# saandeepa93/distributed_compute_pytorch

Measured on AMD Instinct MI355X. Metric: samples/sec (whole node) ResNet-50 DDP at 1/2/4/8 MI355X; scaling efficiency, higher is better.
Workload: dtype bf16; 1 GPU; model=resnet50, global_batch=1024, per_gpu_batch=1024, grad_accum=1, parallelism=dp1, impl=ours, fused_kernels=True, optimizer=SGD, comm_dtype=fp32, hip_graph=False, grad_to_none=True, backend=rccl, mfma_1x1_gemm=True, image_size=224, channels_last=True, res_prologue=False

## Files before the change

### csrc/fused.cpp

```cpp
#include "fused.h"

#include <cstring>

#include <c10/hip/HIPGuard.h>
#include <c10/hip/HIPStream.h>

#include <map>
#include <tuple>
#include <mutex>

#include "common.h"
#include "kernels/bn_kernels.h"
#include "kernels/gemm_kernels.h"
#include "kernels/attn_kernels.h"
#include "kernels/kernels.h"
#include "kernels/ln_kernels.h"
#include "kernels/dropout_kernels.h"
#include "kernels/pool_kernels.h"
#include "kernels/metrics_kernels.h"
#include "kernels/gelu_kernels.h"

namespace dcp {
namespace fused {

// ... 25 lines not shown

struct ZeroArena {
  at::Tensor buf;
  int64_t used = 0;
};
std::mutex g_arena_mu;
std::map<std::pair<int, hipStream_t>, ZeroArena> g_arenas;
constexpr int64_t kArenaFloats = int64_t(4) << 20;

at::Tensor zeroed_floats(int64_t n, const at::Tensor& like, hipStream_t st) {
  hipStreamCaptureStatus cap = hipStreamCaptureStatusNone;
  (void)hipStreamIsCapturing(st, &cap);
  const int64_t need = (n + 63) / 64 * 64;
  if (cap != hipStreamCaptureStatusNone || need > kArenaFloats / 4) {
    return at::zeros({need}, like.options().dtype(at::kFloat)).narrow(0, 0, n);
  }
  std::lock_guard<std::mutex> g(g_arena_mu);
  ZeroArena& a = g_arenas[{static_cast<int>(like.get_device()), st}];
  if (!a.buf.defined()) {
    a.buf = at::empty({kArenaFloats}, like.options().dtype(at::kFloat));
    DK_CHECK(hipMemsetAsync(a.buf.data_ptr(), 0, sizeof(float) * kArenaFloats, st) == hipSuccess, "memset failed");
  }
  if (a.used + need > kArenaFloats) {
    DK_CHECK(hipMemsetAsync(a.buf.data_ptr(), 0, sizeof(float) * kArenaFloats, st) == hipSuccess, "memset failed");
    a.used = 0;
  }
  at::Tensor t = a.buf.narrow(0, a.used, n);
  a.used += need;
  return t;
}

at::Tensor zeroed_vec(int64_t n, const at::Tensor& like, hipStream_t st) {
  constexpr int64_t kSlab = int64_t(1) << 18;
  hipStreamCaptureStatus cap = hipStreamCaptureStatusNone;
  (void)hipStreamIsCapturing(st, &cap);
  const int64_t need = (n + 63) / 64 * 64;
  static const bool off = std::getenv("DCP_NO_GRAD_SLAB") != nullptr;
  if (off || need > kSlab / 4) return at::zeros({n}, like.options().dtype(at::kFloat));
  static std::mutex mu;
  if (cap != hipStreamCaptureStatusNone) {
    unsigned long long id = 0;
    (void)hipStreamGetCaptureInfo(st, &cap, &id);
    static std::map<std::pair<int, hipStream_t>, std::tuple<at::Tensor, int64_t, unsigned long long>> cslabs;
    std::lock_guard<std::mutex> g(mu);
    auto& e = cslabs[{static_cast<int>(like.get_device()), st}];
    if (!std::get<0>(e).defined() || std::get<2>(e) != id || std::get<1>(e) + need > kSlab) {
// ... 643 lines not shown
            "conv1x1_dgrad_resred: mean must be fp32 [N]");
  DK_CHECK(bits.scalar_type() == at::kByte && bits.numel() == M * N / 8 && bits.is_contiguous(),
            "conv1x1_dgrad_resred: relu bits mismatch");
  at::Tensor g2;
  if (gy2.has_value() && gy2->defined()) {
    g2 = gy2->to(at::kBFloat16).contiguous(x.dim() == 4 ? at::MemoryFormat::ChannelsLast : at::MemoryFormat::Contiguous);
    DK_CHECK(g2.sizes() == x.sizes(), "conv1x1_dgrad_resred: gy2 shape");
  }
  const bool has_x2 = x2.has_value() && x2->defined();
  if (has_x2) {
    check_gemm_act(*x2, "conv1x1_dgrad_resred(x2)");
    DK_CHECK(x2->sizes() == x.sizes(), "conv1x1_dgrad_resred: x2 shape");
    DK_CHECK(mean2.has_value() && mean2->defined() && mean2->scalar_type() == at::kFloat && mean2->numel() == N,
              "conv1x1_dgrad_resred: mean2 must be fp32 [N]");
  }
  at::Tensor g = at::empty_like(x, x.dim() == 4 ? at::MemoryFormat::ChannelsLast : at::MemoryFormat::Contiguous);
  auto s = stream_of(gy);
  at::Tensor acc = zeroed_floats(2 * N, gy, s);
  at::Tensor acc2 = has_x2 ? zeroed_floats(2 * N, gy, s) : at::empty({0}, gy.options().dtype(at::kFloat));
  kern::gemm_nt_resred_bf16(gy.data_ptr(), wt.data_ptr(), g.data_ptr(), M, static_cast<int>(N), static_cast<int>(K),
                            x.data_ptr(), mean.data_ptr<float>(), g2.defined() ? g2.data_ptr() : nullptr,
                            bits.data_ptr<uint8_t>(), acc.data_ptr<float>(), has_x2 ? x2->data_ptr() : nullptr,
                            has_x2 ? mean2->data_ptr<float>() : nullptr, has_x2 ? acc2.data_ptr<float>() : nullptr, s);
  return {g, acc, acc2};
}

std::vector<at::Tensor> conv3_bwd_fused(const at::Tensor& g, const at::Tensor& z3, const at::Tensor& gamma3,
                                        const at::Tensor& mean3, const at::Tensor& invstd3, const at::Tensor& acc3,
                                        const at::Tensor& wt, const at::Tensor& x2,
                                        const c10::optional<at::Tensor>& gamma2,
                                        const c10::optional<at::Tensor>& beta2, const at::Tensor& mean2,
                                        const at::Tensor& invstd2) {
  check_gemm_act(g, "conv3_bwd_fused");
  check_gemm_act(z3, "conv3_bwd_fused");
  c10::hip::HIPGuard guard(g.device().index());
  DK_CHECK(g.dim() == 4 && g.sizes() == z3.sizes(), "conv3_bwd_fused: g must match z3");
  const int64_t C = g.size(1);
  const int64_t M = g.numel() / C;
  const int64_t w = C / 4;
  DK_CHECK(C % 4 == 0 && kern::conv3_bwd_mode(M, static_cast<int>(w)) > 0, "conv3_bwd_fused: unsupported shape");
  DK_CHECK(wt.scalar_type() == at::kBFloat16 && wt.is_contiguous() && wt.numel() == w * C,
            "conv3_bwd_fused: weight must be contiguous bf16 [w][4w]");
  auto f32c = [&](const at::Tensor& t, int64_t n) {
    return t.scalar_type() == at::kFloat && t.numel() == n && t.is_contiguous() && t.device() == g.device();
  };
  DK_CHECK(f32c(gamma3, C) && f32c(mean3, C) && f32c(invstd3, C) && f32c(acc3, 2 * C),
// ... 1077 lines not shown
        pybind11::arg("accumulate_into") = pybind11::none());
  m.def("flash_attn_fwd", &flash_attn_fwd, "MFMA flash attention forward (head dim 64)", pybind11::arg("q"),
        pybind11::arg("k"), pybind11::arg("v"), pybind11::arg("heads"), pybind11::arg("causal"),
        pybind11::arg("p_drop"), pybind11::arg("seed"), pybind11::arg("keep_bits") = true,
        pybind11::arg("key_mask") = pybind11::none(), pybind11::kw_only(),
        pybind11::arg("seed_offset") = pybind11::none());
  m.def("flash_attn_bwd", &flash_attn_bwd, "MFMA flash attention backward into dq/dk/dv", pybind11::arg("dout"),
        pybind11::arg("q"), pybind11::arg("k"), pybind11::arg("v"), pybind11::arg("o"), pybind11::arg("lse"),
        pybind11::arg("keep"), pybind11::arg("heads"), pybind11::arg("causal"), pybind11::arg("p_drop"),
        pybind11::arg("seed"), pybind11::arg("dq"), pybind11::arg("dk"), pybind11::arg("dv"),
        pybind11::arg("key_mask") = pybind11::none());
  m.def("attn_pack_key_mask", &attn_pack_key_mask,
        "bool [B, T] key-padding mask -> packed int64 [B, 1 + T/64] for flash_attn_fwd / flash_attn_bwd",
        pybind11::arg("mask"));
  m.def("conv_fwd", &conv_fwd, "kxk NHWC conv forward (implicit-GEMM MFMA) [+ output BN sums]", pybind11::arg("x"),
        pybind11::arg("wt"), pybind11::arg("kh"), pybind11::arg("kw"), pybind11::arg("stride"), pybind11::arg("pad"),
        pybind11::arg("stats") = false);
  m.def("conv1x1_dgrad_bnred", &conv1x1_dgrad_bnred, "1x1 data gradient + BN/ReLU backward reduction epilogue");
  m.def("conv_dgrad_bnred", &conv_dgrad_bnred, "stride-1 kxk data gradient + BN/ReLU backward reduction epilogue");
  m.def("conv1x1_dgrad_resred", &conv1x1_dgrad_resred,
        "1x1 data gradient + residual BN(+RBN)/ReLU backward reduction epilogue -> (g, acc, acc2)",
        pybind11::arg("gy"), pybind11::arg("wt"), pybind11::arg("x"), pybind11::arg("gy2"), pybind11::arg("mean"),
        pybind11::arg("bits"), pybind11::arg("x2") = pybind11::none(), pybind11::arg("mean2") = pybind11::none());
  m.def("bn_bwd_apply_g", &bn_bwd_apply_g, "BN training backward apply from a masked gradient + its reduction");
  m.def("conv3_bwd_fused", &conv3_bwd_fused,
        "bottleneck conv3 backward with BN3's backward apply as its prologue -> (dy2, acc2, dz3)");
  m.def("conv3_bwd_mode", [](int64_t M, int64_t w) { return kern::conv3_bwd_mode(M, static_cast<int>(w)); },
        "0: conv3's backward of this shape stays unfused; 1: conv3_bwd_fused");
  m.def("conv3_bwd_ds_fused", &conv3_bwd_ds_fused,
        "conv3_bwd_fused at a downsample block: both BNs' backward applies as the prologue -> "
        "(dy2, acc2, dz3, dzd[, dxd])");
  m.def("conv3_bwd_ds_mode", [](int64_t M, int64_t w) { return kern::conv3_bwd_ds_mode(M, static_cast<int>(w)); },
        "0: a downsample block of this shape stays on bn_bwd_apply2_g; 1: conv3_bwd_ds_fused without dxd; 2: with");
  m.def("bn_dparams", &bn_dparams, "(dweight, dbias) of a training BN from its backward reduction");
  m.def("conv1_fwd_fused", &conv1_fwd_fused,
        "block boundary relu(bn3(z3) + residual-or-bn_d(x2)) with the next conv1 fed from the same tile -> "
        "(y, bits, z1, sums1, mean, invstd[, mean2, invstd2])",
        pybind11::arg("z3"), pybind11::arg("w"), pybind11::arg("weight"), pybind11::arg("bias"),
        pybind11::arg("running_mean"), pybind11::arg("running_var"), pybind11::arg("num_batches_tracked"),
        pybind11::arg("stats"), pybind11::arg("momentum"), pybind11::arg("eps"),
        pybind11::arg("residual") = pybind11::none(), pybind11::arg("x2") = pybind11::none(),
        pybind11::arg("weight2") = pybind11::none(), pybind11::arg("bias2") = pybind11::none(),
        pybind11::arg("running_mean2") = pybind11::none(), pybind11::arg("running_var2") = pybind11::none(),
        pybind11::arg("num_batches_tracked2") = pybind11::none(), pybind11::arg("stats2") = pybind11::none(),
        pybind11::arg("momentum2") = 0.0, pybind11::arg("eps2") = 0.0);
  m.def("conv1_fwd_mode",
// ... 38 lines not shown
```

### csrc/kernels/gemm.hip

```cpp
#include <hip/hip_runtime.h>

#include <cstdlib>
#include <string>

#include "bf16_vec.h"
#include "gelu_math.h"
#include "gemm_kernels.h"
#include "kernels.h"
#include "stem_kernels.h"

namespace dcp {
namespace kern {
namespace {

typedef short s16x4 __attribute__((ext_vector_type(4)));
typedef short s16x8 __attribute__((ext_vector_type(8)));
typedef __attribute__((address_space(3))) s16x4 lds_s16x4;

constexpr int kT = 256;
int g_wg_slots = 512;
int g_wg_cap = 0;
constexpr int kBK = 32;
constexpr int kNS = 4;

// ... 1568 lines not shown
  const char* v = getenv("DCP_RESERVE_CUS");
  const int r = v ? atoi(v) : 0;
  return r < 0 ? 0 : (r > 192 ? 192 : r);
}();
inline int grid_cus() { return 256 - g_reserve_cus; }
}
void gemm_tune(const char* key, int value) {
  const std::string k(key);
  if (k == "nt_big") g_nt_big = value;
  if (k == "lin_big") g_lin_big = value;
  if (k == "big_pipe") g_big_pipe = value;
  if (k == "nt_a") g_nt_a = value < 0 ? 0 : (value > 3 ? 3 : value);
  if (k == "stem_wide") g_stem_wide = value;
  if (k == "slab32") g_slab32 = value;
  if (k == "nt_deep") g_nt_deep = value;
  if (k == "pro_pipe") g_pro_pipe = value;
  if (k == "wg_slots") g_wg_slots = value < 64 ? 64 : value;
  if (k == "wg_cap") g_wg_cap = value < 0 ? 0 : value;
  if (k == "reserve_cus") g_reserve_cus = value < 0 ? 0 : (value > 192 ? 192 : value);
  if (k.rfind("pp_", 0) == 0) gemm_pp_tune(key, value);
  if (k.rfind("bn_", 0) == 0) bn_tune(key, value);
  if (k.rfind("c3bwd", 0) == 0) conv3_bwd_tune(key, value);
  if (k.rfind("c1fwd", 0) == 0) conv1_fwd_tune(key, value);
  wgrad_pp_tune(key, value);
}
int gemm_tune_get(const char* key) {
  const std::string k(key);
  if (k == "nt_big") return g_nt_big;
  if (k == "lin_big") return g_lin_big;
  if (k == "big_pipe") return g_big_pipe;
  if (k == "nt_a") return g_nt_a;
  if (k == "stem_wide") return g_stem_wide;
  if (k == "slab32") return g_slab32;
  if (k == "nt_deep") return g_nt_deep;
  if (k == "pro_pipe") return g_pro_pipe;
  if (k == "wg_slots") return g_wg_slots;
  if (k == "wg_cap") return g_wg_cap;
  if (k == "reserve_cus") return g_reserve_cus;
  if (k.rfind("pp_", 0) == 0) return gemm_pp_tune_get(key);
  if (k.rfind("bn_", 0) == 0) return bn_tune_get(key);
  if (k.rfind("c3bwd", 0) == 0) return conv3_bwd_tune_get(key);
  if (k.rfind("c1fwd", 0) == 0) return conv1_fwd_tune_get(key);
  return wgrad_pp_tune_get(key);
}

namespace {
template <bool GATHER, int BK, int BM>
void gemm_nt_launch_bm(const void* A, const void* B, void* C, int64_t M, int N, int K, const float* scale,
                       const float* shift, bool relu, float* stats, const ConvGeo& geo, const BnRedArgs* red,
                       hipStream_t s, bool scatter2, bool parity) {
  const int BN = N % 128 == 0 ? 128 : 64;
  const int tiles_m = static_cast<int>((M + BM - 1) / BM);
  const int tn = N / BN;
  const int kRes = (BM == 128 ? 2 : 1) * grid_cus();
  const int64_t tiles = static_cast<int64_t>(tiles_m) * tn;
  int P = tiles <= kRes ? static_cast<int>(tiles) : (kRes / tn) * tn;
  if (P < tn) P = tn;
  const dim3 grid(P);
  const bool pro = scale != nullptr;
  const bool st = stats != nullptr;
  const int nw = (BM / 64) * (BN == 64 && BM == 256 ? 1 : 2);
  const size_t lds = static_cast<size_t>(nt_stages<BK>()) * (BM + BN) * BK * 2 +
                     static_cast<size_t>(nw) * 32 * (BN * 2 / (BM == 256 && BN == 64 ? 1 : 2)) +
                     (pro ? 8 * static_cast<size_t>(K) : 0);
  const int NT = 64 * nw;
// ... 831 lines not shown
```

### csrc/kernels/kernels.h

```cpp
#pragma once

#include <hip/hip_runtime.h>

#include <cstdint>

namespace dcp {
namespace kern {

enum DType : int { F32 = 0, BF16 = 1, F16 = 2 };

constexpr int64_t kChunk = 8192;

struct TableView {
  const int64_t* base;
  int n;
};

void mt_copy(TableView t, int64_t nchunks, DType src, DType dst, float scale, hipStream_t s);

void mt_sgd(TableView t, int64_t nchunks, DType p, float lr, float momentum, float dampening, float wd,
            bool nesterov, bool maximize, bool first_step, bool has_buf, float grad_scale, hipStream_t s);

void mt_adam(TableView t, int64_t nchunks, DType p, float lr, float beta1, float beta2, float eps, float wd,
             float bias_c1, float bias_c2_sqrt, bool amsgrad, bool decoupled_wd, bool maximize, float grad_scale,
// ... 15 lines not shown

void conv3_bwd_bf16(const void* g, const void* z3, const void* wt, const void* x2, void* dz3, void* dy2, int64_t M,
                    int w, const float* gamma3, const float* mean3, const float* invstd3, const float* acc3,
                    const float* gamma2, const float* beta2, const float* mean2, const float* invstd2, float* stats,
                    hipStream_t s);
int conv3_bwd_mode(int64_t M, int w);
void conv3_bwd_ds_bf16(const void* g, const void* z3, const void* zd, const void* wt, const void* wdt, const void* x2,
                       void* dz3, void* dzd, void* dy2, void* dxd, int64_t M, int w, const float* gamma3,
                       const float* mean3, const float* invstd3, const float* acc3, const float* gammad,
                       const float* meand, const float* invstdd, const float* accd, const float* gamma2,
                       const float* beta2, const float* mean2, const float* invstd2, float* stats, hipStream_t s);
int conv3_bwd_ds_mode(int64_t M, int w);
bool conv3_bwd_tune(const char* key, int value);
int conv3_bwd_tune_get(const char* key);
void bn_dparams(const float* acc, const float* invstd, float* dgamma, float* dbeta, int C, hipStream_t s);

void conv1_fwd_bf16(const void* z3, const void* res, const void* w, void* y, uint8_t* bits, void* z1, int64_t M, int K,
                    int N, const float* scale, const float* shift, const float* rscale, const float* rshift,
                    float* stats, hipStream_t s);
int conv1_fwd_mode(int64_t M, int K, int N);
bool conv1_fwd_tune(const char* key, int value);
int conv1_fwd_tune_get(const char* key);

}
}
```

### csrc/selftest/kern_stubs.cpp

```cpp
#include <cstdio>
#include <cstdlib>

#include "kernels/kernels.h"

namespace dcp {
namespace kern {
namespace {
[[noreturn]] void gpu_only(const char* f) {
  std::fprintf(stderr, "%s: GPU launcher reached from a CPU self-test\n", f);
  std::abort();
}
}

void mt_copy(TableView, int64_t, DType, DType, float, hipStream_t) { gpu_only("mt_copy"); }
void mt_sgd(TableView, int64_t, DType, float, float, float, float, bool, bool, bool, bool, float, hipStream_t) {
  gpu_only("mt_sgd");
}
void mt_adam(TableView, int64_t, DType, float, float, float, float, float, float, float, bool, bool, bool, float, bool,
             int, hipStream_t) {
  gpu_only("mt_adam");
}
void mt_adadelta(TableView, int64_t, DType, float, float, float, float, bool, float, hipStream_t) {
  gpu_only("mt_adadelta");
}
// ... 3 lines not shown
void conv3_bwd_bf16(const void*, const void*, const void*, const void*, void*, void*, int64_t, int, const float*,
                    const float*, const float*, const float*, const float*, const float*, const float*, const float*,
                    float*, hipStream_t) {
  gpu_only("conv3_bwd_bf16");
}
int conv3_bwd_mode(int64_t, int) { return 0; }
void conv3_bwd_ds_bf16(const void*, const void*, const void*, const void*, const void*, const void*, void*, void*,
                       void*, void*, int64_t, int, const float*, const float*, const float*, const float*,
                       const float*, const float*, const float*, const float*, const float*, const float*,
                       const float*, const float*, float*, hipStream_t) {
  gpu_only("conv3_bwd_ds_bf16");
}
int conv3_bwd_ds_mode(int64_t, int) { return 0; }
bool conv3_bwd_tune(const char*, int) { return false; }
int conv3_bwd_tune_get(const char*) { return -1; }
void bn_dparams(const float*, const float*, float*, float*, int, hipStream_t) { gpu_only("bn_dparams"); }
void conv1_fwd_bf16(const void*, const void*, const void*, void*, uint8_t*, void*, int64_t, int, int, const float*,
                    const float*, const float*, const float*, float*, hipStream_t) {
  gpu_only("conv1_fwd_bf16");
}
int conv1_fwd_mode(int64_t, int, int) { return 0; }
bool conv1_fwd_tune(const char*, int) { return false; }
int conv1_fwd_tune_get(const char*) { return -1; }

}
}
```

### distributed_compute_pytorch_amd/ops/conv.py

```python
from __future__ import annotations

from typing import Optional, Tuple

import torch
import torch.nn.functional as F

from .._ext import C as _C


def _cl(t: torch.Tensor) -> torch.Tensor:
    if t.dtype != torch.bfloat16:
        t = t.to(torch.bfloat16)
    return t.contiguous(memory_format=torch.channels_last) if t.dim() == 4 else t.contiguous()


_PREPPED = {}


class ConvWeightPrep:

    def __init__(self, weights):
        self.weights = list(weights)
        self._key = None

# ... 175 lines not shown
def _c3_defer_ok(z3: torch.Tensor) -> bool:
    fn = _c3_node(z3)
    c = z3.shape[1]
    if fn is None or _C.conv3_bwd_mode(z3.numel() // c, c // 4) <= 0:
        return False
    fn._c3_defer = True
    return True


def _c3ds_defer_ok(z3: torch.Tensor, zd: torch.Tensor):
    fn, fd = _c3_node(z3), zd.grad_fn
    if (fn is None or fd is None or fd is fn or not _APPLY2 or zd.shape != z3.shape or zd.dtype != z3.dtype
            or not zd.is_contiguous(memory_format=torch.channels_last)):
        return None
    c = z3.shape[1]
    mode = _C.conv3_bwd_ds_mode(z3.numel() // c, c // 4)
    if mode == 2:
        if not isinstance(fd, _Conv1x1Fn._backward_cls) or tuple(fd.wshape) != (c, c // 4, 1, 1):
            return None
    elif mode != 1 or not isinstance(fd, (_Conv1x1Fn._backward_cls, _ConvKxKGemmFn._backward_cls)):
        return None
    fn._c3ds = fd._c3ds = True
    return fn, fd, mode == 2


_PRO_RED = True


class _BNReluConv1x1Fn(torch.autograd.Function):
    @staticmethod
    def forward(ctx, x, gamma, beta, weight, running_mean, running_var, nbt, momentum, eps, stats, sums):
        mean, invstd, scale, shift = _C.bn_stats_coef(x, gamma, beta, running_mean, running_var, float(momentum),
                                                      float(eps), nbt, sums)
        w, wt = _w2d(weight)
        z, st = _C.conv1x1_fwd(x, w, scale, shift, True, bool(stats))
        ctx.save_for_backward(x, gamma, beta, wt, mean, invstd, scale, shift)
        ctx.wshape, ctx.wdtype = weight.shape, weight.dtype
        ctx.mark_non_differentiable(st)
        ctx.set_materialize_grads(False)
        return z, st

    @staticmethod
    def backward(ctx, gz, _gst):
        x, gamma, beta, wt, mean, invstd, scale, shift = ctx.saved_tensors
        if gz is None:
            return (None,) * 11
# ... 84 lines not shown
            w, wt = _w2d(w_next)
            z1, s1 = _C.conv1x1_fwd(y, w, None, None, False, True)
        elif RES_PROLOGUE:
            mean, invstd, scale, shift = _C.bn_stats_coef(z3, gamma, beta, rm, rv, float(momentum), float(eps), nbt,
                                                          stats)
            w, wt = _w2d(w_next)
            z1, s1, y, bits = _C.conv1x1_fwd_res(z3, w, scale, shift, _cl(residual), True)
            mean2 = invstd2 = None
        else:
            y, mean, invstd, bits = _C.bn_act_fwd(z3, gamma, beta, rm, rv, residual, True, float(momentum),
                                                  float(eps), True, nbt, stats)
            mean2 = invstd2 = None
            w, wt = _w2d(w_next)
            z1, s1 = _C.conv1x1_fwd(y, w, None, None, False, True)
        ctx.save_for_backward(z3, gamma, mean, invstd, bits, y, wt, x2, gamma2, mean2, invstd2)
        ctx.wshape, ctx.wdtype = w_next.shape, w_next.dtype
        ctx.mark_non_differentiable(s1)
        return y, z1, s1

    @staticmethod
    def backward(ctx, gy, gz, _gs):
        z3, gamma, mean, invstd, bits, y, wt, x2, gamma2, mean2, invstd2 = ctx.saved_tensors
        if gz is None:
            gz = torch.zeros((y.shape[0], ctx.wshape[0]) + tuple(y.shape[2:]), device=y.device, dtype=y.dtype)
        gz = _cl(gz)
        dw = _C.conv1x1_wgrad(gz, y)
        g, acc, acc2 = _C.conv1x1_dgrad_resred(gz, wt, z3, None if gy is None else _cl(gy), mean, bits, x2, mean2)
        dres = dx2 = dgamma2 = dbeta2 = None
        if x2 is not None and _APPLY2 and ctx.defer_ds:
            _c3ds_put(g, (z3, gamma, mean, invstd, acc, x2, gamma2, mean2, invstd2, acc2), ctx.defer_ds)
            dz3 = dx2 = g
            dgamma, dbeta = _C.bn_dparams(acc, invstd)
            dgamma2, dbeta2 = _C.bn_dparams(acc2, invstd2)
        elif x2 is not None and _APPLY2:
            dz3, dgamma, dbeta, dx2, dgamma2, dbeta2 = _C.bn_bwd_apply2_g(g, z3, gamma, mean, invstd, acc, x2, gamma2,
                                                                          mean2, invstd2, acc2)
        elif ctx.defer:
            _c3_put(g, z3, gamma, mean, invstd, acc)
            dz3 = dres = g
            dgamma, dbeta = _C.bn_dparams(acc, invstd)
        else:
            dz3, dgamma, dbeta = _C.bn_bwd_apply_g(g, z3, gamma, mean, invstd, acc)
            if x2 is not None:
                dx2, dgamma2, dbeta2 = _C.bn_bwd_apply_g(g, x2, gamma2, mean2, invstd2, acc2)
            else:
                dres = g
        dw = dw.view(ctx.wshape)
        if dw.dtype != ctx.wdtype:
            dw = dw.to(ctx.wdtype)
        return (dz3, dgamma, dbeta, dres, dx2, dgamma2, dbeta2, dw) + (None,) * 13
# ... 64 lines not shown
        d3 = _c3_take(ctx, gz)
        ds = _c3ds_take(ctx, gz, 0)
        if d3 is not None or ds is not None:
            dy, acc, gz = (_C.conv3_bwd_fused(gz, *d3, wt, x, gamma, beta, mean, invstd) if d3 is not None
                           else ds[:3])
            dw = _C.conv1x1_wgrad(gz, y).view(wshape)
        elif k == 1 and stride == 1:
            dw = _C.conv1x1_wgrad(gz, y).view(wshape)
            dy, acc = _C.conv1x1_dgrad_bnred(gz, wt, x, gamma, beta, mean, invstd)
        else:
            dw = _C.conv_wgrad(gz, y, k, k, stride, pad)
            if stride == 1:
                wd = wt if wt is not None else w.flip(2, 3).permute(1, 2, 3, 0).contiguous()
                dy, acc = _C.conv_dgrad_bnred(gz, wd, k, k, k - 1 - pad, x, gamma, beta, mean, invstd)
            else:
                dy = torch.ops.aten.convolution_backward(gz, y, w, None, [stride, stride], [pad, pad], [1, 1],
                                                         False, [0, 0], 1, [True, False, False])[0]
                dy = _cl(dy)
                acc = None
        if dw.dtype != wdtype:
            dw = dw.to(wdtype)
        if acc is None:
            dx, dgamma, dbeta, _ = _C.bn_act_bwd(dy, None, x, gamma, beta, mean, invstd, y, True, False, True, None)
        else:
            dx, dgamma, dbeta = _C.bn_act_bwd_apply(dy, x, gamma, beta, mean, invstd, acc)
        return dx, dgamma, dbeta, dw, None, None, None, None, None, None, None, None, None, None


def bn_relu_conv(x: torch.Tensor, bn, weight: torch.Tensor, k: int, stride: int, pad: int,
                 sums: Optional[torch.Tensor] = None, stats: bool = False):
    nbt = bn.num_batches_tracked
    if nbt is not None and (nbt.device != x.device or nbt.dtype != torch.int64):
        nbt.add_(1)
        nbt = None
    return _BNReluConvFn.apply(x, bn.weight, bn.bias, weight, bn.running_mean, bn.running_var, nbt, bn.momentum,
                               bn.eps, sums, k, stride, pad, stats)


class _ConvKxKFn(torch.autograd.Function):

    @staticmethod
    def forward(ctx, x, weight, stride, padding):
        w = weight.detach().to(torch.bfloat16)
        y = F.conv2d(x, w, None, stride, padding)
        ctx.save_for_backward(x, w)
        ctx.stride, ctx.padding, ctx.wdtype = stride, padding, weight.dtype
        return y

    @staticmethod
    def backward(ctx, gy):
        x, w = ctx.saved_tensors
        gy = _cl(gy)
        s, p = ctx.stride, ctx.padding
        dx = None
        if ctx.needs_input_grad[0]:
            dx = torch.ops.aten.convolution_backward(gy, x, w, None, [s, s], [p, p], [1, 1], False, [0, 0], 1,
                                                     [True, False, False])[0]
        dw = None
        if ctx.needs_input_grad[1]:
# ... 92 lines not shown
```

Baseline: 15650 samples/s.

## Add streaming conv1 backward kernel with optional deferred BN1 apply prologue

Adds a new row-tile streaming MFMA kernel for the 1x1 conv1 data gradient at bottleneck boundaries. It fuses the residual BN/ReLU reduction epilogue and can take BN1's backward apply as a prologue, deferring that apply from the bn_relu_conv node through a Python-side handoff. The aim is fewer kernel launches and fewer activation round-trips through HBM in the backward pass. BN1 fusion is off by default (g_bn1=0), so only the streaming dgrad kernel runs for the 64x256 and 128x512 shapes. The arena reset now reallocates its buffer instead of re-zeroing in place, which avoids overwriting slices still in use at the cost of an extra allocation.

```diff
diff --git a/csrc/fused.cpp b/csrc/fused.cpp
--- a/csrc/fused.cpp
+++ b/csrc/fused.cpp
@@ -71,6 +71,7 @@
     DK_CHECK(hipMemsetAsync(a.buf.data_ptr(), 0, sizeof(float) * kArenaFloats, st) == hipSuccess, "memset failed");
   }
   if (a.used + need > kArenaFloats) {
+    a.buf = at::empty({kArenaFloats}, like.options().dtype(at::kFloat));
     DK_CHECK(hipMemsetAsync(a.buf.data_ptr(), 0, sizeof(float) * kArenaFloats, st) == hipSuccess, "memset failed");
     a.used = 0;
   }
@@ -760,6 +761,75 @@
                             x.data_ptr(), mean.data_ptr<float>(), g2.defined() ? g2.data_ptr() : nullptr,
                             bits.data_ptr<uint8_t>(), acc.data_ptr<float>(), has_x2 ? x2->data_ptr() : nullptr,
                             has_x2 ? mean2->data_ptr<float>() : nullptr, has_x2 ? acc2.data_ptr<float>() : nullptr, s);
+  return {g, acc, acc2};
+}
+
+std::vector<at::Tensor> conv1_bwd_fused(const at::Tensor& gy, const at::Tensor& wt, const at::Tensor& x,
+                                        const c10::optional<at::Tensor>& gy2, const at::Tensor& mean,
+                                        const at::Tensor& bits, const c10::optional<at::Tensor>& x2,
+                                        const c10::optional<at::Tensor>& mean2, const c10::optional<at::Tensor>& z1,
+                                        const c10::optional<at::Tensor>& gamma1,
+                                        const c10::optional<at::Tensor>& beta1,
+                                        const c10::optional<at::Tensor>& mean1,
+                                        const c10::optional<at::Tensor>& invstd1,
+                                        const c10::optional<at::Tensor>& acc1) {
+  check_gemm_act(gy, "conv1_bwd_fused");
+  check_gemm_act(x, "conv1_bwd_fused");
+  c10::hip::HIPGuard guard(gy.device().index());
+  DK_CHECK(gy.dim() == 4 && x.dim() == 4, "conv1_bwd_fused: gy and x must be channels_last 4-D tensors");
+  const int64_t K = gy.size(1), N = x.size(1);
+  const int64_t M = gy.numel() / K;
+  const int mode = kern::conv1_bwd_mode(M, static_cast<int>(K), static_cast<int>(N));
+  DK_CHECK(mode > 0, "conv1_bwd_fused: unsupported shape");
+  DK_CHECK(wt.scalar_type() == at::kBFloat16 && wt.is_contiguous() && wt.numel() == N * K &&
+                wt.device() == gy.device(),
+            "conv1_bwd_fused: weight must be contiguous bf16 [N][K]");
+  DK_CHECK(x.numel() == M * N && x.size(0) == gy.size(0) && x.device() == gy.device(), "conv1_bwd_fused: x shape");
+  auto f32c = [&](const at::Tensor& t, int64_t n) {
+    return t.scalar_type() == at::kFloat && t.numel() == n && t.is_contiguous() && t.device() == gy.device();
+  };
+  DK_CHECK(f32c(mean, N), "conv1_bwd_fused: mean must be fp32 [N]");
+  DK_CHECK(bits.scalar_type() == at::kByte && bits.numel() == M * N / 8 && bits.is_contiguous() &&
+                bits.device() == gy.device(),
+            "conv1_bwd_fused: relu bits mismatch");
+  at::Tensor g2;
+  if (gy2.has_value() && gy2->defined()) {
+    g2 = gy2->to(at::kBFloat16).contiguous(at::MemoryFormat::ChannelsLast);
+    DK_CHECK(g2.sizes() == x.sizes() && g2.device() == gy.device(), "conv1_bwd_fused: gy2 shape");
+  }
+  const bool has_x2 = x2.has_value() && x2->defined();
+  if (has_x2) {
+    check_gemm_act(*x2, "conv1_bwd_fused(x2)");
+    DK_CHECK(x2->sizes() == x.sizes() && x2->device() == gy.device(), "conv1_bwd_fused: x2 shape");
+    DK_CHECK(mean2.has_value() && mean2->defined() && f32c(*mean2, N), "conv1_bwd_fused: mean2 must be fp32 [N]");
+  }
+  const bool bn1 = z1.has_value() && z1->defined();
+  BnRedIn r1;
+  if (bn1) {
+    DK_CHECK(mode == 2, "conv1_bwd_fused: BN1 fusion is switched off (gemm_tune c1bwd_bn1)");
+    DK_CHECK(mean1.has_value() && mean1->defined() && invstd1.has_value() && invstd1->defined() &&
+                  acc1.has_value() && acc1->defined() && f32c(*mean1, K) && f32c(*invstd1, K) && f32c(*acc1, 2 * K),
+              "conv1_bwd_fused: BN1 mean / invstd fp32 [K], acc fp32 [2*K]");
+    r1 = bnred_in(*z1, gamma1, beta1, *mean1, *invstd1, K, "conv1_bwd_fused(z1)");
+    DK_CHECK(z1->sizes() == gy.sizes() && z1->device() == gy.device(), "conv1_bwd_fused: z1 must match gy");
+    DK_CHECK((!r1.w.defined() || f32c(r1.w, K)) && (!r1.b.defined() || f32c(r1.b, K)),
+              "conv1_bwd_fused: BN1 gamma / beta [K]");
+  }
+  at::Tensor g = at::empty_like(x, at::MemoryFormat::ChannelsLast);
+  at::Tensor dz1;
+  if (bn1) dz1 = at::empty_like(gy, at::MemoryFormat::ChannelsLast);
+  auto s = stream_of(gy);
+  at::Tensor acc = zeroed_floats(2 * N, gy, s);
+  at::Tensor acc2 = has_x2 ? zeroed_floats(2 * N, gy, s) : at::empty({0}, gy.options().dtype(at::kFloat));
+  kern::conv1_bwd_bf16(gy.data_ptr(), wt.data_ptr(), g.data_ptr(), M, static_cast<int>(N), static_cast<int>(K),
+                       x.data_ptr(), mean.data_ptr<float>(), g2.defined() ? g2.data_ptr() : nullptr,
+                       bits.data_ptr<uint8_t>(), acc.data_ptr<float>(), has_x2 ? x2->data_ptr() : nullptr,
+                       has_x2 ? mean2->data_ptr<float>() : nullptr, has_x2 ? acc2.data_ptr<float>() : nullptr,
+                       bn1 ? z1->data_ptr() : nullptr, bn1 && r1.w.defined() ? r1.w.data_ptr<float>() : nullptr,
+                       bn1 && r1.b.defined() ? r1.b.data_ptr<float>() : nullptr, bn1 ? r1.mean : nullptr,
+                       bn1 ? r1.invstd : nullptr, bn1 ? acc1->data_ptr<float>() : nullptr,
+                       bn1 ? dz1.data_ptr() : nullptr, s);
+  if (bn1) return {g, acc, acc2, dz1};
   return {g, acc, acc2};
 }
 
@@ -1883,6 +1953,18 @@
         "1x1 data gradient + residual BN(+RBN)/ReLU backward reduction epilogue -> (g, acc, acc2)",
         pybind11::arg("gy"), pybind11::arg("wt"), pybind11::arg("x"), pybind11::arg("gy2"), pybind11::arg("mean"),
         pybind11::arg("bits"), pybind11::arg("x2") = pybind11::none(), pybind11::arg("mean2") = pybind11::none());
+  m.def("conv1_bwd_fused", &conv1_bwd_fused,
+        "conv1x1_dgrad_resred on the streaming row-tile kernel -> (g, acc, acc2); with z1 … acc1 BN1's backward "
+        "apply is its prologue (gy = dy1) -> (g, acc, acc2, dz1)",
+        pybind11::arg("gy"), pybind11::arg("wt"), pybind11::arg("x"), pybind11::arg("gy2"), pybind11::arg("mean"),
+        pybind11::arg("bits"), pybind11::arg("x2") = pybind11::none(), pybind11::arg("mean2") = pybind11::none(),
+        pybind11::arg("z1") = pybind11::none(), pybind11::arg("gamma1") = pybind11::none(),
+        pybind11::arg("beta1") = pybind11::none(), pybind11::arg("mean1") = pybind11::none(),
+        pybind11::arg("invstd1") = pybind11::none(), pybind11::arg("acc1") = pybind11::none());
+  m.def("conv1_bwd_mode",
+        [](int64_t M, int64_t K, int64_t N) { return kern::conv1_bwd_mode(M, static_cast<int>(K), static_cast<int>(N)); },
+        "0: conv1's boundary data gradient of this shape stays on conv1x1_dgrad_resred; 1: conv1_bwd_fused; "
+        "2: and BN1's backward apply may be deferred into it");
   m.def("bn_bwd_apply_g", &bn_bwd_apply_g, "BN training backward apply from a masked gradient + its reduction");
   m.def("conv3_bwd_fused", &conv3_bwd_fused,
         "bottleneck conv3 backward with BN3's backward apply as its prologue -> (dy2, acc2, dz3)");
diff --git a/csrc/kernels/conv1_bwd.hip b/csrc/kernels/conv1_bwd.hip
--- /dev/null
+++ b/csrc/kernels/conv1_bwd.hip
@@ -0,0 +1,346 @@
+#include <hip/hip_runtime.h>
+
+#include <cstring>
+
+#include "bf16_vec.h"
+#include "kernels.h"
+
+namespace dcp {
+namespace kern {
+namespace {
+
+constexpr int kBM = 32;
+
+int g_mode64 = 1;
+int g_mode128 = 1;
+int g_mode128x256 = 0;
+int g_bn1 = 0;
+int g_grid = 0;
+
+struct C1BArgs {
+  const uint16_t* a;
+  const uint16_t* z1;
+  uint16_t* dz1;
+  const uint16_t* wt;
+  const uint16_t* z3;
+  const uint16_t* gy2;
+  const uint8_t* bits;
+  const uint16_t* x2;
+  uint16_t* g;
+  const float* mean3;
+  const float* meand;
+  float* acc;
+  float* acc2;
+  const float* gamma1;
+  const float* beta1;
+  const float* mean1;
+  const float* invstd1;
+  const float* acc1;
+  int64_t M;
+  int tiles;
+};
+
+template <int K, int N, bool X2, bool BN1>
+__global__ void __launch_bounds__(4 * K, 2) conv1_bwd_kernel(const C1BArgs a) {
+  constexpr int T = 4 * K;
+  constexpr int NW = T / 64;
+  constexpr int WN = N / NW;
+  constexpr int FN = WN / 16;
+  constexpr int FM = kBM / 16;
+  constexpr int KS = K / 32;
+  constexpr int ACH = K / 8;
+  constexpr int CPR = N / 8;
+  constexpr int RPP = T / CPR;
+  constexpr int NP = kBM / RPP;
+  static_assert(T == kBM * ACH && RPP * NP == kBM && FN * 16 * NW == N && CPR >= 16, "tile shape");
+  __shared__ __attribute__((aligned(16))) char sA[kBM * K * 2];
+  __shared__ __attribute__((aligned(16))) char sC[kBM * N * 2];
+  static_assert(RPP * N * 4 <= kBM * N * 2, "sums fit the staging image");
+  __shared__ __attribute__((aligned(16))) float sK[BN1 ? 6 * K : 4];
+
+  const int t = threadIdx.x, lane = t & 63, wv = t >> 6;
+  const int cc = t % CPR, r0 = t / CPR;
+  const int ach = t % ACH, arow = t / ACH;
+  const int64_t M = a.M;
+  const bool has2 = a.gy2 != nullptr;
+
+  const int P = gridDim.x, wg = xcd_remap(blockIdx.x, P);
+
+  if constexpr (BN1) {
+    for (int c = t; c < K; c += T) {
+      const float inv = a.invstd1[c];
+      const float sb = a.acc1[c], sg = a.acc1[K + c];
+      const float m = a.mean1[c];
+      const float sc = (a.gamma1 ? a.gamma1[c] : 1.f) * inv;
+      sK[c] = sc;
+      sK[K + c] = sb / static_cast<float>(M);
+      sK[2 * K + c] = sg / static_cast<float>(M) * inv * inv;
+      sK[3 * K + c] = m;
+      sK[4 * K + c] = sc;
+      sK[5 * K + c] = (a.beta1 ? a.beta1[c] : 0.f) - m * sc;
+    }
+    __syncthreads();
+  }
+  bf16x8 wf[FN][KS];
+#pragma unroll
+  for (int i = 0; i < FN; ++i) {
+    const uint16_t* wp = a.wt + static_cast<int64_t>(WN * wv + 16 * i + (lane & 15)) * K + 8 * (lane >> 4);
+#pragma unroll
+    for (int ks = 0; ks < KS; ++ks) wf[i][ks] = *reinterpret_cast<const bf16x8*>(wp + 32 * ks);
+  }
+  float rmu[8], rmu2[X2 ? 8 : 1], ssum[8], ssq[8], ss2[X2 ? 8 : 1];
+#pragma unroll
+  for (int k = 0; k < 8; ++k) {
+    rmu[k] = a.mean3[cc * 8 + k];
+    if constexpr (X2) {
+      rmu2[k] = a.meand[cc * 8 + k];
+      ss2[k] = 0.f;
+    }
+    ssum[k] = ssq[k] = 0.f;
+  }
+
+  uint4 aq, zq1;
+  auto load_a = [&](int tl) {
+    const int64_t m0 = static_cast<int64_t>(tl) * kBM;
+    const int rem = static_cast<int>(M - m0 < kBM ? M - m0 : kBM);
+    const uint32_t lo = (arow < rem ? arow : 0) * K + ach * 8;
+    aq = ld16_nt(a.a + m0 * K + lo);
+    if constexpr (BN1) zq1 = ld16_nt(a.z1 + m0 * K + lo);
+  };
+  uint4 zq[NP], gq[NP], xq[X2 ? NP : 1];
+  uint32_t bq[NP];
+  auto load_e = [&](int tl, int i) {
+    const int64_t m0 = static_cast<int64_t>(tl) * kBM;
+    const int rem = static_cast<int>(M - m0 < kBM ? M - m0 : kBM);
+    const int row = r0 + RPP * i;
+    const uint32_t lo = (row < rem ? row : 0) * N + cc * 8;
+    zq[i] = ld16_nt(a.z3 + m0 * N + lo);
+    if (has2) gq[i] = ld16_nt(a.gy2 + m0 * N + lo);
+    bq[i] = __builtin_nontemporal_load(a.bits + (m0 * N >> 3) + (lo >> 3));
+    if constexpr (X2) xq[i] = ld16_nt(a.x2 + m0 * N + lo);
+  };
+#pragma unroll
+  for (int i = 0; i < NP; ++i) gq[i] = make_uint4(0, 0, 0, 0);
+
+  int tl = wg;
+  if (tl < a.tiles) {
+    load_a(tl);
+#pragma unroll
+    for (int i = 0; i < NP; ++i) load_e(tl, i);
+  }
+  for (; tl < a.tiles; tl += P) {
+    const int64_t m0 = static_cast<int64_t>(tl) * kBM;
+    const bool more = tl + P < a.tiles;
+    {
+      uint4 v = aq;
+      if constexpr (BN1) {
+        const uint32_t g4[4] = {aq.x, aq.y, aq.z, aq.w};
+        const uint32_t z4[4] = {zq1.x, zq1.y, zq1.z, zq1.w};
+        float k1[8], k2[8], k3[8], mu[8], sc[8], sf[8], d[8];
+#pragma unroll
+        for (int h = 0; h < 2; ++h) {
+          const float* kp = sK + ach * 8 + 4 * h;
+          *reinterpret_cast<float4*>(k1 + 4 * h) = *reinterpret_cast<const float4*>(kp);
+          *reinterpret_cast<float4*>(k2 + 4 * h) = *reinterpret_cast<const float4*>(kp + K);
+          *reinterpret_cast<float4*>(k3 + 4 * h) = *reinterpret_cast<const float4*>(kp + 2 * K);
+          *reinterpret_cast<float4*>(mu + 4 * h) = *reinterpret_cast<const float4*>(kp + 3 * K);
+          *reinterpret_cast<float4*>(sc + 4 * h) = *reinterpret_cast<const float4*>(kp + 4 * K);
+          *reinterpret_cast<float4*>(sf + 4 * h) = *reinterpret_cast<const float4*>(kp + 5 * K);
+        }
+#pragma unroll
+        for (int k = 0; k < 8; ++k) {
+          float gk = (k & 1) ? bf_hi(g4[k >> 1]) : bf_lo(g4[k >> 1]);
+          const float xk = (k & 1) ? bf_hi(z4[k >> 1]) : bf_lo(z4[k >> 1]);
+          gk = fmaf(xk, sc[k], sf[k]) > 0.f ? gk : 0.f;
+          d[k] = k1[k] * (gk - k2[k] - (xk - mu[k]) * k3[k]);
+        }
+        v = make_uint4(pack2(d[0], d[1]), pack2(d[2], d[3]), pack2(d[4], d[5]), pack2(d[6], d[7]));
+        if (m0 + arow < M) st16_nt(a.dz1 + (m0 + arow) * K + ach * 8, v);
+      }
+      if (m0 + arow >= M) v = make_uint4(0, 0, 0, 0);
+      const int sw = ACH >= 16 ? (arow & 15) : ((arow >> 1) & 7);
+      *reinterpret_cast<uint4*>(sA + arow * (K * 2) + 16 * (ach ^ sw)) = v;
+    }
+    __syncthreads();
+    if (more) load_a(tl + P);
+
+    f32x4 acc[FN][FM];
+#pragma unroll
+    for (int i = 0; i < FN; ++i)
+#pragma unroll
+      for (int j = 0; j < FM; ++j) acc[i][j] = f32x4{0.f, 0.f, 0.f, 0.f};
+#pragma unroll
+    for (int ks = 0; ks < KS; ++ks) {
+      bf16x8 xf[FM];
+#pragma unroll
+      for (int j = 0; j < FM; ++j) {
+        const int row = 16 * j + (lane & 15);
+        const int sw = ACH >= 16 ? (row & 15) : ((row >> 1) & 7);
+        xf[j] = *reinterpret_cast<const bf16x8*>(sA + row * (K * 2) + 16 * ((4 * ks + (lane >> 4)) ^ sw));
+      }
+#pragma unroll
+      for (int i = 0; i < FN; ++i)
+#pragma unroll
+        for (int j = 0; j < FM; ++j)
+          acc[i][j] = __builtin_amdgcn_mfma_f32_16x16x32_bf16(wf[i][ks], xf[j], acc[i][j], 0, 0, 0);
+    }
+#pragma unroll
+    for (int j = 0; j < FM; ++j) {
+      const int row = 16 * j + (lane & 15);
+#pragma unroll
+      for (int i = 0; i < FN; ++i) {
+        const int col = WN * wv + 16 * i + 4 * (lane >> 4);
+        *reinterpret_cast<uint2*>(sC + row * (N * 2) + 16 * ((col >> 3) ^ (row & 15)) + (col & 7) * 2) =
+            make_uint2(pack2(acc[i][j][0], acc[i][j][1]), pack2(acc[i][j][2], acc[i][j][3]));
+      }
+    }
+    __syncthreads();
+
+#pragma unroll
+    for (int i = 0; i < NP; ++i) {
+      const int row = r0 + RPP * i;
+      const int64_t m = m0 + row;
+      const uint4 v = *reinterpret_cast<const uint4*>(sC + row * (N * 2) + 16 * (cc ^ (row & 15)));
+      if (m < M) {
+        const uint32_t w4[4] = {v.x, v.y, v.z, v.w}, y4[4] = {gq[i].x, gq[i].y, gq[i].z, gq[i].w};
+        const uint32_t x4[4] = {zq[i].x, zq[i].y, zq[i].z, zq[i].w};
+        const uint32_t mb = bq[i];
+        float gk[8];
+#pragma unroll
+        for (int k = 0; k < 8; ++k) {
+          const float av = (k & 1) ? bf_hi(w4[k >> 1]) : bf_lo(w4[k >> 1]);
+          const float bv = (k & 1) ? bf_hi(y4[k >> 1]) : bf_lo(y4[k >> 1]);
+          const float xk = (k & 1) ? bf_hi(x4[k >> 1]) : bf_lo(x4[k >> 1]);
+          gk[k] = (mb >> k) & 1u ? av + bv : 0.f;
+          ssum[k] += gk[k];
+          ssq[k] = fmaf(gk[k], xk - rmu[k], ssq[k]);
+        }
+        if constexpr (X2) {
+          const uint32_t z4[4] = {xq[i].x, xq[i].y, xq[i].z, xq[i].w};
+#pragma unroll
+          for (int k = 0; k < 8; ++k) {
+            const float zk = (k & 1) ? bf_hi(z4[k >> 1]) : bf_lo(z4[k >> 1]);
+            ss2[k] = fmaf(gk[k], zk - rmu2[k], ss2[k]);
+          }
+        }
+        st16_nt(a.g + m * N + cc * 8,
+                make_uint4(pack2(gk[0], gk[1]), pack2(gk[2], gk[3]), pack2(gk[4], gk[5]), pack2(gk[6], gk[7])));
+      }
+      if (more) load_e(tl + P, i);
+    }
+  }
+
+  float* red = reinterpret_cast<float*>(sC);
+#pragma unroll
+  for (int s = 0; s < (X2 ? 3 : 2); ++s) {
+    __syncthreads();
+#pragma unroll
+    for (int h = 0; h < 2; ++h) {
+      float4 o = make_float4(0.f, 0.f, 0.f, 0.f);
+      if (s == 0) o = make_float4(ssum[4 * h], ssum[4 * h + 1], ssum[4 * h + 2], ssum[4 * h + 3]);
+      else if (s == 1) o = make_float4(ssq[4 * h], ssq[4 * h + 1], ssq[4 * h + 2], ssq[4 * h + 3]);
+      else if constexpr (X2) o = make_float4(ss2[4 * h], ss2[4 * h + 1], ss2[4 * h + 2], ss2[4 * h + 3]);
+      *reinterpret_cast<float4*>(red + r0 * N + cc * 8 + 4 * h) = o;
+    }
+    __syncthreads();
+    for (int c = t; c < N; c += T) {
+      float v = 0.f;
+#pragma unroll
+      for (int r = 0; r < RPP; ++r) v += red[r * N + c];
+      if (s == 0) {
+        atomicAdd(a.acc + c, v);
+        if constexpr (X2) atomicAdd(a.acc2 + c, v);
+      } else if (s == 1) {
+        atomicAdd(a.acc + N + c, v);
+      } else if constexpr (X2) {
+        atomicAdd(a.acc2 + N + c, v);
+      }
+    }
+  }
+}
+
+int* mode_of(int K, int N) {
+  if (K == 64 && N == 256) return &g_mode64;
+  if (K == 128 && N == 512) return &g_mode128;
+  if (K == 128 && N == 256) return &g_mode128x256;
+  return nullptr;
+}
+
+template <int K, int N>
+void launch(const C1BArgs& a, int per_cu, hipStream_t s) {
+  int P = 256 * per_cu;
+  if (g_grid > 0 && g_grid < P) P = g_grid;
+  if (P > a.tiles) P = a.tiles;
+  const bool x2 = a.x2 != nullptr, bn1 = a.z1 != nullptr;
+  if (x2 && bn1) hipLaunchKernelGGL((conv1_bwd_kernel<K, N, true, true>), dim3(P), dim3(4 * K), 0, s, a);
+  else if (x2) hipLaunchKernelGGL((conv1_bwd_kernel<K, N, true, false>), dim3(P), dim3(4 * K), 0, s, a);
+  else if (bn1) hipLaunchKernelGGL((conv1_bwd_kernel<K, N, false, true>), dim3(P), dim3(4 * K), 0, s, a);
+  else hipLaunchKernelGGL((conv1_bwd_kernel<K, N, false, false>), dim3(P), dim3(4 * K), 0, s, a);
+}
+
+}
+
+bool conv1_bwd_tune(const char* key, int value) {
+  const int m = value < 0 ? 0 : (value > 1 ? 1 : value);
+  if (!strcmp(key, "c1bwd")) g_mode64 = g_mode128 = g_mode128x256 = m;
+  else if (!strcmp(key, "c1bwd64")) g_mode64 = m;
+  else if (!strcmp(key, "c1bwd128")) g_mode128 = m;
+  else if (!strcmp(key, "c1bwd128x256")) g_mode128x256 = m;
+  else if (!strcmp(key, "c1bwd_bn1")) g_bn1 = m;
+  else if (!strcmp(key, "c1bwd_grid")) g_grid = value < 0 ? 0 : value;
+  else return false;
+  return true;
+}
+
+int conv1_bwd_tune_get(const char* key) {
+  if (!strcmp(key, "c1bwd")) {
+    const int m = g_mode64 < g_mode128 ? g_mode64 : g_mode128;
+    return m < g_mode128x256 ? m : g_mode128x256;
+  }
+  if (!strcmp(key, "c1bwd64")) return g_mode64;
+  if (!strcmp(key, "c1bwd128")) return g_mode128;
+  if (!strcmp(key, "c1bwd128x256")) return g_mode128x256;
+  if (!strcmp(key, "c1bwd_bn1")) return g_bn1;
+  if (!strcmp(key, "c1bwd_grid")) return g_grid;
+  return -1;
+}
+
+int conv1_bwd_mode(int64_t M, int K, int N) {
+  if (M <= 0 || M >= (int64_t(1) << 31)) return 0;
+  const int* m = mode_of(K, N);
+  if (!m || *m <= 0) return 0;
+  return g_bn1 ? 2 : 1;
+}
+
+void conv1_bwd_bf16(const void* a, const void* wt, void* g, int64_t M, int N, int K, const void* z3,
+                    const float* mean3, const void* gy2, const uint8_t* bits, float* acc, const void* x2,
+                    const float* mean2, float* acc2, const void* z1, const float* gamma1, const float* beta1,
+                    const float* mean1, const float* invstd1, const float* acc1, void* dz1, hipStream_t s) {
+  C1BArgs r;
+  r.a = static_cast<const uint16_t*>(a);
+  r.z1 = static_cast<const uint16_t*>(z1);
+  r.dz1 = static_cast<uint16_t*>(dz1);
+  r.wt = static_cast<const uint16_t*>(wt);
+  r.z3 = static_cast<const uint16_t*>(z3);
+  r.gy2 = static_cast<const uint16_t*>(gy2);
+  r.bits = bits;
+  r.x2 = static_cast<const uint16_t*>(x2);
+  r.g = static_cast<uint16_t*>(g);
+  r.mean3 = mean3;
+  r.meand = mean2;
+  r.acc = acc;
+  r.acc2 = acc2;
+  r.gamma1 = gamma1;
+  r.beta1 = beta1;
+  r.mean1 = mean1;
+  r.invstd1 = invstd1;
+  r.acc1 = acc1;
+  r.M = M;
+  r.tiles = static_cast<int>((M + kBM - 1) / kBM);
+  if (K == 64 && N == 256) launch<64, 256>(r, 2, s);
+  else if (K == 128 && N == 512) launch<128, 512>(r, 1, s);
+  else launch<128, 256>(r, 1, s);
+}
+
+}
+}
diff --git a/csrc/kernels/gemm.hip b/csrc/kernels/gemm.hip
--- a/csrc/kernels/gemm.hip
+++ b/csrc/kernels/gemm.hip
@@ -1614,6 +1614,7 @@
   if (k.rfind("bn_", 0) == 0) bn_tune(key, value);
   if (k.rfind("c3bwd", 0) == 0) conv3_bwd_tune(key, value);
   if (k.rfind("c1fwd", 0) == 0) conv1_fwd_tune(key, value);
+  if (k.rfind("c1bwd", 0) == 0) conv1_bwd_tune(key, value);
   wgrad_pp_tune(key, value);
 }
 int gemm_tune_get(const char* key) {
@@ -1633,6 +1634,7 @@
   if (k.rfind("bn_", 0) == 0) return bn_tune_get(key);
   if (k.rfind("c3bwd", 0) == 0) return conv3_bwd_tune_get(key);
   if (k.rfind("c1fwd", 0) == 0) return conv1_fwd_tune_get(key);
+  if (k.rfind("c1bwd", 0) == 0) return conv1_bwd_tune_get(key);
   return wgrad_pp_tune_get(key);
 }
 
diff --git a/csrc/kernels/kernels.h b/csrc/kernels/kernels.h
--- a/csrc/kernels/kernels.h
+++ b/csrc/kernels/kernels.h
@@ -61,5 +61,13 @@
 bool conv1_fwd_tune(const char* key, int value);
 int conv1_fwd_tune_get(const char* key);
 
+void conv1_bwd_bf16(const void* a, const void* wt, void* g, int64_t M, int N, int K, const void* z3,
+                    const float* mean3, const void* gy2, const uint8_t* bits, float* acc, const void* x2,
+                    const float* mean2, float* acc2, const void* z1, const float* gamma1, const float* beta1,
+                    const float* mean1, const float* invstd1, const float* acc1, void* dz1, hipStream_t s);
+int conv1_bwd_mode(int64_t M, int K, int N);
+bool conv1_bwd_tune(const char* key, int value);
+int conv1_bwd_tune_get(const char* key);
+
 }
 }
diff --git a/csrc/selftest/kern_stubs.cpp b/csrc/selftest/kern_stubs.cpp
--- a/csrc/selftest/kern_stubs.cpp
+++ b/csrc/selftest/kern_stubs.cpp
@@ -49,6 +49,14 @@
 int conv1_fwd_mode(int64_t, int, int) { return 0; }
 bool conv1_fwd_tune(const char*, int) { return false; }
 int conv1_fwd_tune_get(const char*) { return -1; }
+void conv1_bwd_bf16(const void*, const void*, void*, int64_t, int, int, const void*, const float*, const void*,
+                    const uint8_t*, float*, const void*, const float*, float*, const void*, const float*, const float*,
+                    const float*, const float*, const float*, void*, hipStream_t) {
+  gpu_only("conv1_bwd_bf16");
+}
+int conv1_bwd_mode(int64_t, int, int) { return 0; }
+bool conv1_bwd_tune(const char*, int) { return false; }
+int conv1_bwd_tune_get(const char*) { return -1; }
 
 }
 }
diff --git a/distributed_compute_pytorch_amd/ops/conv.py b/distributed_compute_pytorch_amd/ops/conv.py
--- a/distributed_compute_pytorch_amd/ops/conv.py
+++ b/distributed_compute_pytorch_amd/ops/conv.py
@@ -221,6 +221,55 @@
         return None
     fn._c3ds = fd._c3ds = True
     return fn, fd, mode == 2
+
+
+_C1_DEFERRED: dict = {}
+
+
+def _c1_put(dy: torch.Tensor, z1, gamma, beta, mean, invstd, acc) -> None:
+    if _C1_DEFERRED:
+        _C1_DEFERRED.clear()
+        raise RuntimeError("conv1 backward fusion: a deferred BN1 gradient of an earlier node was never taken by its "
+                           "block boundary node (gemm_tune c1bwd_bn1=0 disables the fusion)")
+    _C1_DEFERRED[dy.data_ptr()] = (dy, z1, gamma, beta, mean, invstd, acc)
+
+
+def _c1_take(ctx, gz: torch.Tensor):
+    if not _c1_marked(ctx):
+        return None
+    e = _C1_DEFERRED.pop(gz.data_ptr(), None)
+    if e is None or e[0].shape != gz.shape or e[0].dtype != gz.dtype:
+        _C1_DEFERRED.clear()
+        raise RuntimeError("conv1 backward fusion: this boundary's z1 was handed to a node that defers BN1's backward "
+                           "apply, but the gradient it received is not that node's deferred one (z1 has another "
+                           "consumer?); gemm_tune c1bwd_bn1=0 disables the fusion")
+    return e[1:]
+
+
+def _c1_shape_mode(m: int, k: int, n: int, dtype: torch.dtype, channels_last: bool) -> int:
+    if dtype != torch.bfloat16 or not channels_last:
+        return 0
+    return int(_C.conv1_bwd_mode(m, k, n))
+
+
+def _c1_mark(z1: torch.Tensor, z: torch.Tensor, affine: bool) -> None:
+    fb, fn = z1.grad_fn, z.grad_fn
+    if fb is None or fn is None or not isinstance(fb, _BNResActConv1x1Fn._backward_cls) or z1.output_nr != 1:
+        return
+    mark = getattr(fb, "_c1_bn1", None)
+    if mark is not None:
+        mark[0] = False
+        return
+    k, n = z1.shape[1], fb.wshape[1]
+    on = (affine and fn.cfg[0] == 3 and fn.cfg[1] == 1 and z1.dim() == 4
+          and _c1_shape_mode(z1.numel() // k, k, n, z1.dtype,
+                             z1.is_contiguous(memory_format=torch.channels_last)) == 2)
+    fb._c1_bn1 = fn._c1_bn1 = [on]
+
+
+def _c1_marked(ctx) -> bool:
+    mark = getattr(ctx, "_c1_bn1", None)
+    return mark is not None and mark[0]
 
 
 _PRO_RED = True
@@ -351,10 +400,23 @@
     def backward(ctx, gy, gz, _gs):
         z3, gamma, mean, invstd, bits, y, wt, x2, gamma2, mean2, invstd2 = ctx.saved_tensors
         if gz is None:
-            gz = torch.zeros((y.shape[0], ctx.wshape[0]) + tuple(y.shape[2:]), device=y.device, dtype=y.dtype)
-        gz = _cl(gz)
-        dw = _C.conv1x1_wgrad(gz, y)
-        g, acc, acc2 = _C.conv1x1_dgrad_resred(gz, wt, z3, None if gy is None else _cl(gy), mean, bits, x2, mean2)
+            gz = _cl(torch.zeros((y.shape[0], ctx.wshape[0]) + tuple(y.shape[2:]), device=y.device, dtype=y.dtype))
+            bn1 = None
+        else:
+            gz = _cl(gz)
+            bn1 = _c1_take(ctx, gz)
+        gy2 = None if gy is None else _cl(gy)
+        k, n = gz.shape[1], z3.shape[1]
+        if bn1 is not None:
+            g, acc, acc2, gz = _C.conv1_bwd_fused(gz, wt, z3, gy2, mean, bits, x2, mean2, *bn1)
+            dw = _C.conv1x1_wgrad(gz, y)
+        else:
+            dw = _C.conv1x1_wgrad(gz, y)
+            if z3.dim() == 4 and gz.dtype == z3.dtype and _c1_shape_mode(
+                    gz.numel() // k, k, n, z3.dtype, z3.is_contiguous(memory_format=torch.channels_last)) > 0:
+                g, acc, acc2 = _C.conv1_bwd_fused(gz, wt, z3, gy2, mean, bits, x2, mean2)
+            else:
+                g, acc, acc2 = _C.conv1x1_dgrad_resred(gz, wt, z3, gy2, mean, bits, x2, mean2)
         dres = dx2 = dgamma2 = dbeta2 = None
         if x2 is not None and _APPLY2 and ctx.defer_ds:
             _c3ds_put(g, (z3, gamma, mean, invstd, acc, x2, gamma2, mean2, invstd2, acc2), ctx.defer_ds)
@@ -465,6 +527,10 @@
             dw = dw.to(wdtype)
         if acc is None:
             dx, dgamma, dbeta, _ = _C.bn_act_bwd(dy, None, x, gamma, beta, mean, invstd, y, True, False, True, None)
+        elif _c1_marked(ctx):
+            _c1_put(dy, x, gamma, beta, mean, invstd, acc)
+            dx = dy
+            dgamma, dbeta = _C.bn_dparams(acc, invstd)
         else:
             dx, dgamma, dbeta = _C.bn_act_bwd_apply(dy, x, gamma, beta, mean, invstd, acc)
         return dx, dgamma, dbeta, dw, None, None, None, None, None, None, None, None, None, None
@@ -476,8 +542,10 @@
     if nbt is not None and (nbt.device != x.device or nbt.dtype != torch.int64):
         nbt.add_(1)
         nbt = None
-    return _BNReluConvFn.apply(x, bn.weight, bn.bias, weight, bn.running_mean, bn.running_var, nbt, bn.momentum,
-                               bn.eps, sums, k, stride, pad, stats)
+    z, st = _BNReluConvFn.apply(x, bn.weight, bn.bias, weight, bn.running_mean, bn.running_var, nbt, bn.momentum,
+                                bn.eps, sums, k, stride, pad, stats)
+    _c1_mark(x, z, bn.weight is not None and bn.bias is not None)
+    return z, st
 
 
 class _ConvKxKFn(torch.autograd.Function):
```

Result: no change. 15770 samples/s, median of 6 (+0.7%).
